# PKU-VCL-Geometry/GeoSplatting

Measured on AMD Instinct MI355X. Metric: fwd+bwd views/sec at 2M Gaussians, 800x800, higher is better.
Workload: dtype f32

## Files before the change

geosplatting_amd/csrc/gs_segsort_dev.h:

```cpp
#pragma once
#include <stdint.h>

#ifndef GS_SEGSORT_FN
#define GS_SEGSORT_FN __device__ __forceinline__
#endif

typedef unsigned long long gs_u64;

template <bool PAD>
GS_SEGSORT_FN int gs_seg_phys(int i) { return PAD ? i + (i >> 5) : i; }

template <bool F64>
GS_SEGSORT_FN gs_u64 gs_seg_inf() { return F64 ? 0x7ff0000000000000ull : ~0ull; }

template <bool F64>
GS_SEGSORT_FN void gs_seg_cx(gs_u64& a, gs_u64& b)
{
#if defined(__HIP_DEVICE_COMPILE__)
    if (F64) {
        const double x = __builtin_bit_cast(double, a), y = __builtin_bit_cast(double, b);
        double lo, hi;
        asm("v_min_f64 %0, %1, %2" : "=v"(lo) : "v"(x), "v"(y));
        asm("v_max_f64 %0, %1, %2" : "=v"(hi) : "v"(x), "v"(y));
        a = __builtin_bit_cast(gs_u64, lo); b = __builtin_bit_cast(gs_u64, hi);
        return;
    }
#endif
    const gs_u64 lo = a < b ? a : b, hi = a < b ? b : a;
    a = lo; b = hi;
}

template <int F, bool PAD, bool F64, bool GUARD>
GS_SEGSORT_FN void gs_seg_first(gs_u64* buf, int n, int P, int tid, int nthreads)
{
    constexpr int R = 1 << F;
    for (int v = tid; v < (P >> F); v += nthreads) {
        const int base = v << F;
        if (base >= n) break;
        gs_u64 e[R];
#pragma unroll
        for (int r = 0; r < R; ++r) e[r] = (!GUARD || base + r < n) ? buf[gs_seg_phys<PAD>(base + r)] : gs_seg_inf<F64>();
#pragma unroll
        for (int lgk = 1; lgk <= F; ++lgk) {
#pragma unroll
            for (int r = 0; r < R; ++r)
                if (r < (r ^ ((1 << lgk) - 1))) gs_seg_cx<F64>(e[r], e[r ^ ((1 << lgk) - 1)]);
#pragma unroll
            for (int s = lgk - 2; s >= 0; --s) {
#pragma unroll
                for (int r = 0; r < R; ++r)
                    if ((r & (1 << s)) == 0) gs_seg_cx<F64>(e[r], e[r | (1 << s)]);
            }
        }
#pragma unroll
        for (int r = 0; r < R; ++r) if (!GUARD || base + r < n) buf[gs_seg_phys<PAD>(base + r)] = e[r];
    }
}

template <int G, bool PAD, bool F64, bool GUARD>
GS_SEGSORT_FN void gs_seg_group(gs_u64* buf, int n, int P, int a, bool flip, int tid, int nthreads)
{
    constexpr int R = 1 << G, H = R >> 1;
    const int jmask = (1 << a) - 1;
    for (int v = tid; v < (P >> G); v += nthreads) {
        const int base = ((v >> a) << (a + G)) | (v & jmask);
        if (base >= n) break;
        const int base2 = flip ? (base ^ jmask) : base;
        gs_u64 e[R];
#pragma unroll
        for (int r = 0; r < R; ++r) {
            const int i = (r >= H ? base2 : base) + (r << a);
            e[r] = (!GUARD || i < n) ? buf[gs_seg_phys<PAD>(i)] : gs_seg_inf<F64>();
        }
        if (flip) {
#pragma unroll
            for (int r = 0; r < H; ++r) gs_seg_cx<F64>(e[r], e[R - 1 - r]);
        } else {
#pragma unroll
            for (int r = 0; r < H; ++r) gs_seg_cx<F64>(e[r], e[r + H]);
        }
#pragma unroll
        for (int s = G - 2; s >= 0; --s) {
#pragma unroll
            for (int r = 0; r < R; ++r)
                if ((r & (1 << s)) == 0) gs_seg_cx<F64>(e[r], e[r | (1 << s)]);
        }
#pragma unroll
        for (int r = 0; r < R; ++r) {
            const int i = (r >= H ? base2 : base) + (r << a);
            if (!GUARD || i < n) buf[gs_seg_phys<PAD>(i)] = e[r];
        }
    }
}

template <int GMAX, bool PAD, bool F64, bool GUARD>
GS_SEGSORT_FN void gs_seg_group_n(int g, gs_u64* buf, int n, int P, int a, bool flip, int tid, int nthreads)
{
    if (g == GMAX) gs_seg_group<GMAX, PAD, F64, GUARD>(buf, n, P, a, flip, tid, nthreads);
    else if constexpr (GMAX > 1) gs_seg_group_n<GMAX - 1, PAD, F64, GUARD>(g, buf, n, P, a, flip, tid, nthreads);
}

#define GS_SEG_SORT_BODY(GMAX, PAD, F64, GUARD, buf, n, P, tid, nthreads, BARRIER)                           \
    do {                                                                                                     \
        gs_seg_first<GMAX, PAD, F64, GUARD>(buf, n, P, tid, nthreads);                                       \
        BARRIER;                                                                                             \
        for (int k_ = 2 << (GMAX), lgk_ = (GMAX) + 1; k_ <= (P); k_ <<= 1, ++lgk_) {                         \
            int rem_ = lgk_;                                                                                 \
            bool flip_ = true;                                                                               \
            while (rem_ > 0) {                                                                               \
                const int g_ = flip_ ? ((rem_ - 1) % (GMAX)) + 1 : (GMAX);                                   \
                gs_seg_group_n<GMAX, PAD, F64, GUARD>(g_, buf, n, P, rem_ - g_, flip_, tid, nthreads);       \
                BARRIER;                                                                                     \
                rem_ -= g_;                                                                                  \
                flip_ = false;                                                                               \
            }                                                                                                \
        }                                                                                                    \
    } while (0)
```

geosplatting_amd/csrc/gs_sort.hip:

```cpp
#include "gs_common.h"
#include "gs_segsort_dev.h"

#include <cstdlib>
#include <cstring>

#define RS_THREADS 256
#define RS_WAVES 4
#define RS_ITEMS 8
#define RS_TILE (RS_THREADS * RS_ITEMS)
#define RS_WCHUNK (64 * RS_ITEMS)

typedef unsigned long long u64;

static int tile_bits(int tile_w, int tile_h)
{
    unsigned n = (unsigned)(tile_w * tile_h);
    int b = 0;
    while (n > 1) { n >>= 1; ++b; }
    return b + 1;
}

struct PairItem { u64 key; int32_t val; };
struct PairIn {
    const u64* keys; const int32_t* vals;
    __device__ __forceinline__ PairItem load(int64_t i) const { return PairItem{ keys[i], vals[i] }; }
};
struct PairOut {
    u64* keys; int32_t* vals;
    __device__ __forceinline__ void store(int64_t i, const PairItem& it) const { keys[i] = it.key; vals[i] = it.val; }
};
struct PairDigit {
    int shift; unsigned mask;
    __device__ __forceinline__ unsigned operator()(const PairItem& it) const { return (unsigned)(it.key >> shift) & mask; }
};

struct U2In {
    const uint2* p;
    __device__ __forceinline__ uint2 load(int64_t i) const { return p[i]; }
};
struct U2Out {
    uint2* p;
    __device__ __forceinline__ void store(int64_t i, const uint2& it) const { p[i] = it; }
};
struct DepthIn {
    const float* depths;
    __device__ __forceinline__ uint2 load(int64_t i) const { return make_uint2(__float_as_uint(depths[i]), (unsigned)i); }
};
struct XDigit {
    int shift; unsigned mask;
    __device__ __forceinline__ unsigned operator()(const uint2& it) const { return (it.x >> shift) & mask; }
};
struct FinalTiles {
    int32_t* tile_ids; int32_t* flatten_ids;
    __device__ __forceinline__ void store(int64_t i, const uint2& it) const
    {
        flatten_ids[i] = (int32_t)it.y;
        tile_ids[i] = (int32_t)it.x;
    }
};
struct FinalOut {
    u64* isect_ids; int32_t* flatten_ids; const float* depths;
    __device__ __forceinline__ void store(int64_t i, const uint2& it) const
    {
        flatten_ids[i] = (int32_t)it.y;
        isect_ids[i] = ((u64)it.x << 32) | (u64)__float_as_uint(depths[it.y]);
    }
};

template <typename Item, typename In, typename Digit>
__global__ void __launch_bounds__(RS_THREADS)
radix_hist_kernel(GsCount nc, In in, Digit digit, int nbins, int nblocks, unsigned* __restrict__ table)
{
    const int64_t n = gs_count(nc);
    __shared__ unsigned hist[256];
    hist[threadIdx.x] = 0u;
    __syncthreads();
    const int64_t base = (int64_t)blockIdx.x * RS_TILE;
#pragma unroll 4
    for (int k = 0; k < RS_ITEMS; ++k) {
        const int64_t i = base + (int64_t)k * RS_THREADS + threadIdx.x;
        if (i < n) atomicAdd(&hist[digit(in.load(i))], 1u);
    }
    __syncthreads();
    if ((int)threadIdx.x < nbins) table[(size_t)threadIdx.x * nblocks + blockIdx.x] = hist[threadIdx.x];
}

__global__ void __launch_bounds__(256)
radix_rowscan_kernel(int nblocks, unsigned* __restrict__ table, unsigned* __restrict__ row_total)
{
    __shared__ unsigned wsum[4];
    unsigned* row = table + (size_t)blockIdx.x * nblocks;
    const int lane = threadIdx.x & 63, wave = threadIdx.x >> 6;
    unsigned carry = 0u;
    for (int i0 = 0; i0 < nblocks; i0 += 256) {
        const int i = i0 + threadIdx.x;
        const unsigned v = i < nblocks ? row[i] : 0u;
        unsigned incl = v;
        incl = gs_wave_incl_scan(incl);
        if (lane == 63) wsum[wave] = incl;
        __syncthreads();
        unsigned before = 0u, all = 0u;
        for (int w = 0; w < 4; ++w) { if (w < wave) before += wsum[w]; all += wsum[w]; }
        if (i < nblocks) row[i] = carry + before + incl - v;
        carry += all;
        __syncthreads();
    }
    if (threadIdx.x == 0) row_total[blockIdx.x] = carry;
}

template <typename Item, typename In, typename Digit, typename Out, int NBITS>
__global__ void __launch_bounds__(RS_THREADS)
radix_scatter_kernel(GsCount nc, In in, Digit digit, int nblocks, const unsigned* __restrict__ table,
                     const unsigned* __restrict__ row_total, Out out)
{
    const int64_t n = gs_count(nc);
    constexpr int NB = 1 << NBITS;
    __shared__ unsigned cnt[RS_WAVES][NB];
    __shared__ unsigned dstart[NB];
    __shared__ unsigned gbase[NB];
    __shared__ Item stage[RS_TILE];
    const int lane = threadIdx.x & 63, wave = threadIdx.x >> 6;
    for (int i = threadIdx.x; i < RS_WAVES * NB; i += RS_THREADS) (&cnt[0][0])[i] = 0u;
    __syncthreads();
    const int64_t bbase = (int64_t)blockIdx.x * RS_TILE;
    const int64_t wbase = bbase + (int64_t)wave * RS_WCHUNK;
    const int n_here = (n - bbase) < RS_TILE ? (int)((n - bbase) > 0 ? (n - bbase) : 0) : RS_TILE;
    const u64 lane_lt = (1ull << lane) - 1ull;
    Item item[RS_ITEMS];
    unsigned dig[RS_ITEMS];
    unsigned rank[RS_ITEMS];
#pragma unroll
    for (int k = 0; k < RS_ITEMS; ++k) {
        const int64_t i = wbase + (int64_t)k * 64 + lane;
        const bool valid = i < n;
        if (valid) item[k] = in.load(i);
        const unsigned d = valid ? digit(item[k]) : 0u;
        u64 m = __ballot(valid);
#pragma unroll
        for (int b = 0; b < NBITS; ++b) {
            const bool bit = (d >> b) & 1u;
            const u64 bal = __ballot(bit);
            m &= bit ? bal : ~bal;
        }
        const unsigned old = cnt[wave][d];
        __builtin_amdgcn_wave_barrier();
        const unsigned r = __popcll(m & lane_lt);
        if (valid && r == 0u) cnt[wave][d] = old + (unsigned)__popcll(m);
        __builtin_amdgcn_fence(__ATOMIC_RELEASE, "wavefront");
        __builtin_amdgcn_wave_barrier();
        __builtin_amdgcn_fence(__ATOMIC_ACQUIRE, "wavefront");
        dig[k] = d;
        rank[k] = old + r;
    }
    __syncthreads();
    {
        const int d = threadIdx.x;
        unsigned tot = 0u;
        if (d < NB) for (int w = 0; w < RS_WAVES; ++w) tot += cnt[w][d];
        unsigned incl = tot;
        incl = gs_wave_incl_scan(incl);
        __shared__ unsigned wtot[RS_WAVES];
        if (lane == 63) wtot[wave] = incl;
        __syncthreads();
        unsigned before = 0u;
        for (int w = 0; w < wave; ++w) before += wtot[w];
        if (d < NB) dstart[d] = before + incl - tot;
        __syncthreads();
        const unsigned rt = d < NB ? row_total[d] : 0u;
        unsigned rincl = rt;
        rincl = gs_wave_incl_scan(rincl);
        if (lane == 63) wtot[wave] = rincl;
        __syncthreads();
        unsigned rbefore = 0u;
        for (int w = 0; w < wave; ++w) rbefore += wtot[w];
        if (d < NB) gbase[d] = rbefore + rincl - rt + table[(size_t)d * nblocks + blockIdx.x];
    }
    __syncthreads();
#pragma unroll
    for (int k = 0; k < RS_ITEMS; ++k) {
        const int64_t i = wbase + (int64_t)k * 64 + lane;
        if (i < n) {
            const unsigned d = dig[k];
            unsigned off = dstart[d] + rank[k];
            for (int w = 0; w < wave; ++w) off += cnt[w][d];
            stage[off] = item[k];
        }
    }
    __syncthreads();
#pragma unroll 4
    for (int k = 0; k < RS_ITEMS; ++k) {
        const int p = k * RS_THREADS + (int)threadIdx.x;
        if (p < n_here) {
            const Item it = stage[p];
            const unsigned d = digit(it);
            out.store((int64_t)gbase[d] + (int64_t)(p - (int)dstart[d]), it);
        }
    }
}

template <typename Item, typename In, typename Digit, typename Out>
static int radix_pass(GsCount nc, In in, Digit digit, Out out, int nbits, unsigned* table, hipStream_t s)
{
    const int64_t n = nc.n;
    const int nblocks = (int)((n + RS_TILE - 1) / RS_TILE);
    const int nbins = 1 << nbits;
    unsigned* row_total = table + (size_t)256 * nblocks;
    hipLaunchKernelGGL((radix_hist_kernel<Item, In, Digit>), dim3(nblocks), dim3(RS_THREADS), 0, s, nc, in, digit, nbins, nblocks, table);
    GS_CHECK_LAUNCH();
    hipLaunchKernelGGL(radix_rowscan_kernel, dim3(nbins), dim3(256), 0, s, nblocks, table, row_total);
    GS_CHECK_LAUNCH();
    switch (nbits) {
#define RS_CASE(B) case B: hipLaunchKernelGGL((radix_scatter_kernel<Item, In, Digit, Out, B>), dim3(nblocks), dim3(RS_THREADS), 0, s, nc, in, digit, nblocks, table, row_total, out); break;
        RS_CASE(1) RS_CASE(2) RS_CASE(3) RS_CASE(4) RS_CASE(5) RS_CASE(6) RS_CASE(7) RS_CASE(8)
#undef RS_CASE
        default: gs_set_error("radix_pass: bad digit width %d", nbits); return GS_EINVAL;
    }
    GS_CHECK_LAUNCH();
    return GS_OK;
}

static size_t align256(size_t x) { return (x + 255) & ~(size_t)255; }
static size_t table_bytes(int64_t n) { return align256(((size_t)256 * (size_t)((n + RS_TILE - 1) / RS_TILE + 1) + 512) * sizeof(unsigned)); }

extern "C" size_t gs_sort_ws_bytes(int64_t n_isects, int tile_w, int tile_h)
{
    if (n_isects <= 0) return 0;
    (void)tile_w; (void)tile_h;
    return table_bytes(n_isects) + align256((size_t)n_isects * 8) + align256((size_t)n_isects * 4) + 256;
}

extern "C" int gs_isect_sort(int64_t n_isects, const int64_t* isect_ids, const int32_t* flatten_ids,
                             int64_t* isect_ids_sorted, int32_t* flatten_ids_sorted, int tile_w, int tile_h,
                             void* ws, size_t ws_bytes, void* stream)
{
    GS_CHECK_ARG(n_isects >= 0 && tile_w > 0 && tile_h > 0, "bad sizes");
    if (n_isects == 0) return GS_OK;
    GS_CHECK_ARG(ws != nullptr, "workspace must not be NULL");
    if (ws_bytes < gs_sort_ws_bytes(n_isects, tile_w, tile_h)) { gs_set_error("gs_isect_sort: workspace too small"); return GS_ENOSPC; }
    hipStream_t s = (hipStream_t)stream;
    char* p = (char*)ws;
    unsigned* table = (unsigned*)p; p += table_bytes(n_isects);
    u64* tk = (u64*)p; p += align256((size_t)n_isects * 8);
    int32_t* tv = (int32_t*)p;
    const int end_bit = 32 + tile_bits(tile_w, tile_h);
    const int npass = (end_bit + 7) / 8;
    const u64* src_k = (const u64*)isect_ids; const int32_t* src_v = flatten_ids;
    for (int pass = 0; pass < npass; ++pass) {
        const int shift = pass * 8;
        const int nbits = (end_bit - shift) < 8 ? (end_bit - shift) : 8;
        const bool to_out = ((npass - 1 - pass) % 2) == 0;
        u64* dk = to_out ? (u64*)isect_ids_sorted : tk;
        int32_t* dv = to_out ? flatten_ids_sorted : tv;
        const int rc = radix_pass<PairItem>(GsCount{ n_isects, nullptr }, PairIn{ src_k, src_v }, PairDigit{ shift, (1u << nbits) - 1u }, PairOut{ dk, dv }, nbits, table, s);
        if (rc != GS_OK) return rc;
        src_k = dk; src_v = dv;
    }
    return GS_OK;
}

__device__ __forceinline__ void tile_range_sorted(float mx, float my, int radius, int tile_size, int tw, int th,
                                                  int& x0, int& y0, int& x1, int& y1)
{
#pragma clang fp contract(off)
    const float ts = (float)tile_size;
    const float tr = (float)radius / ts;
    const float tx = mx / ts, ty = my / ts;
    const float fx0 = floorf(tx - tr), fy0 = floorf(ty - tr);
    const float fx1 = ceilf(tx + tr), fy1 = ceilf(ty + tr);
    x0 = fx0 < 0.0f ? 0 : (fx0 > (float)tw ? tw : (int)fx0);
    y0 = fy0 < 0.0f ? 0 : (fy0 > (float)th ? th : (int)fy0);
    x1 = fx1 < 0.0f ? 0 : (fx1 > (float)tw ? tw : (int)fx1);
    y1 = fy1 < 0.0f ? 0 : (fy1 > (float)th ? th : (int)fy1);
}

#define EM_THREADS 256
#define EM_PER 4
#define EM_LOOK 4
#define EM_TILE (EM_THREADS * EM_PER)

__global__ void __launch_bounds__(256)
tile_rect_kernel(GsCount vc, const float* __restrict__ means2d, const int32_t* __restrict__ radii, int tile_size, int tile_w, int tile_h,
                 uint2* __restrict__ rect)
{
    const int V = (int)gs_count(vc);
    const int v = blockIdx.x * blockDim.x + threadIdx.x;
    if (v >= V) return;
    const float2 m = *reinterpret_cast<const float2*>(means2d + 2 * (size_t)v);
    int x0 = 0, y0 = 0, x1 = 0, y1 = 0;
    const int r = radii[v];
    if (r > 0) tile_range_sorted(m.x, m.y, r, tile_size, tile_w, tile_h, x0, y0, x1, y1);
    rect[v] = make_uint2((unsigned)x0 | ((unsigned)y0 << 16), (unsigned)x1 | ((unsigned)y1 << 16));
}
__device__ __forceinline__ unsigned rect_count(uint2 q)
{
    const int w = (int)(q.y & 0xffffu) - (int)(q.x & 0xffffu), h = (int)(q.y >> 16) - (int)(q.x >> 16);
    return (w > 0 && h > 0) ? (unsigned)(w * h) : 0u;
}

static size_t bf_state_bytes(int V) { return align256(16 + 2 * (size_t)((V + EM_TILE - 1) / EM_TILE + 1) * sizeof(u64)); }

extern "C" size_t gs_isect_bin_ws_bytes(int V, int64_t n_isects, int tile_w, int tile_h)
{
    (void)tile_w; (void)tile_h;
    const size_t v = V > 0 ? (size_t)V : 1, n = n_isects > 0 ? (size_t)n_isects : 1;
    const size_t tb = table_bytes((int64_t)(v > n ? v : n));
    return tb + 3 * align256(v * 8) + bf_state_bytes((int)v) + 2 * align256(n * 8) + 256;
}

__global__ void capacity_check_kernel(const long long* __restrict__ counts, long long v_cap, long long i_cap, long long* __restrict__ status)
{
    if (threadIdx.x != 0 || blockIdx.x != 0) return;
    const long long V = counts[0], I = counts[1];
    if (V > v_cap || I > i_cap) {
        status[0] = GS_ENOSPC;
        if (I > status[1]) status[1] = I;
        if (V > status[2]) status[2] = V;
    }
}

static int isect_bin_impl(int V, const float* means2d, const int32_t* radii, const float* depths, int64_t n_isects,
                          const long long* counts_dev, int tile_size, int tile_w, int tile_h, int64_t* isect_ids_sorted,
                          int32_t* flatten_ids_sorted, void* ws, size_t ws_bytes, void* stream, int32_t* tile_ids_sorted);

extern "C" int gs_isect_bin(int V, const float* means2d, const int32_t* radii, const float* depths,
                            const int32_t* tiles_per_gauss, int64_t n_isects, int tile_size, int tile_w, int tile_h,
                            int64_t* isect_ids_sorted, int32_t* flatten_ids_sorted, void* ws, size_t ws_bytes, void* stream)
{
    (void)tiles_per_gauss;
    return isect_bin_impl(V, means2d, radii, depths, n_isects, nullptr, tile_size, tile_w, tile_h, isect_ids_sorted, flatten_ids_sorted,
                          ws, ws_bytes, stream, nullptr);
}

extern "C" int gs_isect_bin_cap(int V_cap, const float* means2d, const int32_t* radii, const float* depths, const int64_t* counts_dev,
                                int64_t n_isects_cap, int tile_size, int tile_w, int tile_h, int64_t* isect_ids_sorted,
                                int32_t* flatten_ids_sorted, void* ws, size_t ws_bytes, int64_t* status_dev, void* stream)
{
    GS_CHECK_ARG(counts_dev != nullptr && status_dev != nullptr, "counts_dev / status_dev must not be NULL");
    hipLaunchKernelGGL(capacity_check_kernel, dim3(1), dim3(64), 0, (hipStream_t)stream, (const long long*)counts_dev, (long long)V_cap,
                       (long long)n_isects_cap, (long long*)status_dev);
    GS_CHECK_LAUNCH();
    return isect_bin_impl(V_cap, means2d, radii, depths, n_isects_cap, (const long long*)counts_dev, tile_size, tile_w, tile_h,
                          isect_ids_sorted, flatten_ids_sorted, ws, ws_bytes, stream, nullptr);
}

extern "C" int gs_isect_bin_tiles_cap(int V_cap, const float* means2d, const int32_t* radii, const float* depths, const int64_t* counts_dev,
                                      int64_t n_isects_cap, int tile_size, int tile_w, int tile_h, int32_t* tile_ids_sorted,
                                      int32_t* flatten_ids_sorted, void* ws, size_t ws_bytes, int64_t* status_dev, void* stream)
{
    GS_CHECK_ARG(counts_dev != nullptr && status_dev != nullptr && tile_ids_sorted != nullptr, "counts_dev / status_dev / tile_ids_sorted must not be NULL");
    hipLaunchKernelGGL(capacity_check_kernel, dim3(1), dim3(64), 0, (hipStream_t)stream, (const long long*)counts_dev, (long long)V_cap,
                       (long long)n_isects_cap, (long long*)status_dev);
    GS_CHECK_LAUNCH();
    return isect_bin_impl(V_cap, means2d, radii, depths, n_isects_cap, (const long long*)counts_dev, tile_size, tile_w, tile_h,
                          nullptr, flatten_ids_sorted, ws, ws_bytes, stream, tile_ids_sorted);
}

struct KeyIn {
    const unsigned* keys;
    __device__ __forceinline__ uint2 load(int64_t i) const { return make_uint2(keys[i], (unsigned)i); }
};
#define BF_HIST_MAX 8192

__global__ void __launch_bounds__(256)
bin_setup_kernel(unsigned* __restrict__ state, int n_state_words,
                 const long long* __restrict__ counts, long long v_cap, long long i_cap, long long* __restrict__ status)
{
    const int i = blockIdx.x * blockDim.x + threadIdx.x, stride = gridDim.x * blockDim.x;
    for (int k = i; k < n_state_words; k += stride) state[k] = 0u;
    if (i == 0 && counts != nullptr && status != nullptr) {
        const long long V = counts[0], I = counts[1];
        if (V > v_cap || I > i_cap) {
            status[0] = GS_ENOSPC;
            if (I > status[1]) status[1] = I;
            if (V > status[2]) status[2] = V;
        }
    }
}

#define BF_VALID (1ull << 63)
#define BF_SPIN_LIMIT (1 << 22)

__global__ void __launch_bounds__(EM_THREADS)
emit_chained_kernel(GsCount vc, const uint2* __restrict__ order, const uint2* __restrict__ rect, unsigned* __restrict__ ctrl,
                    u64* __restrict__ desc, int n_blocks, int tile_w, uint2* __restrict__ items, unsigned item_cap,
                    long long* __restrict__ status )
{
    const int V = (int)gs_count(vc);
    __shared__ unsigned ws[EM_THREADS / 64];
    __shared__ unsigned s_block;
    __shared__ unsigned long long s_base;
    const int lane = threadIdx.x & 63, wave = threadIdx.x >> 6;
    if (threadIdx.x == 0) s_block = atomicAdd(ctrl, 1u);
    __syncthreads();
    const int block = (int)s_block;
    u64* agg = desc; u64* pre = desc + n_blocks;
    const int r0 = block * EM_TILE + (int)threadIdx.x * EM_PER;
    int v[EM_PER]; unsigned c[EM_PER]; uint2 q[EM_PER];
    unsigned mine = 0u;
#pragma unroll
    for (int k = 0; k < EM_PER; ++k) {
        const int r = r0 + k;
        v[k] = r < V ? (int)order[r].y : -1;
        q[k] = v[k] >= 0 ? rect[v[k]] : make_uint2(0u, 0u);
        c[k] = rect_count(q[k]);
        mine += c[k];
    }
    unsigned incl = mine;
    incl = gs_wave_incl_scan(incl);
    if (lane == 63) ws[wave] = incl;
    __syncthreads();
    unsigned before = 0u, total = 0u;
    for (int w = 0; w < EM_THREADS / 64; ++w) { if (w < wave) before += ws[w]; total += ws[w]; }
    if (wave == 0) {
        unsigned long long acc = 0ull;
        if (block > 0) {
            if (lane == 0) __hip_atomic_store(&agg[block], (u64)total | BF_VALID, __ATOMIC_RELAXED, __HIP_MEMORY_SCOPE_AGENT);
            int pos = block - 1;
            bool done = false;
            while (!done) {
                u64 pv[EM_LOOK], av[EM_LOOK];
#pragma unroll
                for (int j = 0; j < EM_LOOK; ++j) {
                    const int idx = pos - 64 * j - lane;
                    pv[j] = av[j] = 0ull;
                    if (idx >= 0) {
                        pv[j] = __hip_atomic_load(&pre[idx], __ATOMIC_RELAXED, __HIP_MEMORY_SCOPE_AGENT);
                        av[j] = __hip_atomic_load(&agg[idx], __ATOMIC_RELAXED, __HIP_MEMORY_SCOPE_AGENT);
                    }
                }
#pragma unroll
                for (int j = 0; j < EM_LOOK; ++j) {
                    if (done) break;
                    const int idx = pos - 64 * j - lane;
                    bool isP = idx < 0;
                    u64 val = 0ull;
                    if (idx >= 0) {
                        int spins = 0;
                        for (;;) {
                            if (pv[j] & BF_VALID) { isP = true; val = pv[j]; break; }
                            if (av[j] & BF_VALID) { val = av[j]; break; }
                            if (++spins > BF_SPIN_LIMIT) { atomicExch(ctrl + 1, 1u); if (status) status[0] = GS_ENOSPC; break; }
                            __builtin_amdgcn_s_sleep(2);
                            pv[j] = __hip_atomic_load(&pre[idx], __ATOMIC_RELAXED, __HIP_MEMORY_SCOPE_AGENT);
                            av[j] = __hip_atomic_load(&agg[idx], __ATOMIC_RELAXED, __HIP_MEMORY_SCOPE_AGENT);
                        }
                    }
                    const u64 pmask = __ballot(isP);
                    const int first = pmask ? __builtin_ctzll(pmask) : 64;
                    if (lane <= first) acc += val & ~BF_VALID;
                    if (pmask) done = true;
                }
                pos -= 64 * EM_LOOK;
            }
        }
        const unsigned long long base = gs_wave_sum_u64(acc);
        if (lane == 0) {
            __hip_atomic_store(&pre[block], (u64)(base + total) | BF_VALID, __ATOMIC_RELAXED, __HIP_MEMORY_SCOPE_AGENT);
            s_base = base;
        }
    }
    __syncthreads();
    unsigned long long cur = s_base + before + incl - mine;
#pragma unroll
    for (int k = 0; k < EM_PER; ++k) {
        if (v[k] < 0 || c[k] == 0u) continue;
        const int x0 = (int)(q[k].x & 0xffffu), y0 = (int)(q[k].x >> 16), x1 = (int)(q[k].y & 0xffffu), y1 = (int)(q[k].y >> 16);
        for (int i = y0; i < y1; ++i)
            for (int j = x0; j < x1; ++j) {
                const unsigned t = (unsigned)(i * tile_w + j);
                if (cur < (unsigned long long)item_cap) items[cur] = make_uint2(t, (unsigned)v[k]);
                ++cur;
            }
    }
}

#define SEG_CLASSES 3
#define SEG_CAP0 2048
#define SEG_CAP1 4096
#define SEG_CAP2 16384
#define SEG_GMAX 4
#define SEG_THREADS(cap) ((cap) >> SEG_GMAX > 1024 ? 1024 : ((cap) >> SEG_GMAX))
#define SEG_BINS 64
static size_t seg_lds_bytes(int cap) { return (size_t)(cap + (cap >> 5) + 1) * sizeof(u64); }

extern "C" int gs_isect_bin_front_classes(int* caps, int max)
{
    const int c[SEG_CLASSES] = { SEG_CAP0, SEG_CAP1, SEG_CAP2 };
    for (int i = 0; i < SEG_CLASSES && i < max; ++i) if (caps) caps[i] = c[i];
    return SEG_CLASSES;
}

struct SegLists { unsigned* count; int32_t* lists; };

__device__ __forceinline__ int seg_class(unsigned len) { return len <= SEG_CAP0 ? 0 : (len <= SEG_CAP1 ? 1 : (len <= SEG_CAP2 ? 2 : 3)); }
__device__ __forceinline__ int seg_bin(unsigned len)
{
    const int l2 = 31 - __clz((int)len);
    const int half = l2 > 0 ? (int)((len >> (l2 - 1)) & 1u) : 0;
    return SEG_BINS - 1 - (2 * l2 + half);
}

__global__ void __launch_bounds__(1024)
tile_offsets_scan_kernel(int n_tiles, const unsigned* __restrict__ tile_counts, GsCount nc, int32_t* __restrict__ offsets, SegLists sl)
{
    __shared__ unsigned wsum[16];
    __shared__ unsigned s_bin[(SEG_CLASSES + 1) * SEG_BINS];
    const unsigned n = (unsigned)gs_count(nc);
    const int lane = threadIdx.x & 63, wave = threadIdx.x >> 6;
    if (sl.count && threadIdx.x < (SEG_CLASSES + 1) * SEG_BINS) s_bin[threadIdx.x] = 0u;
    __syncthreads();
    unsigned carry = 0u;
    for (int i0 = 0; i0 < n_tiles; i0 += 1024) {
        const int i = i0 + threadIdx.x;
        const unsigned v = i < n_tiles ? tile_counts[i] : 0u;
        unsigned incl = v;
        incl = gs_wave_incl_scan(incl);
        if (lane == 63) wsum[wave] = incl;
        __syncthreads();
        unsigned before = 0u, all = 0u;
        for (int w = 0; w < 16; ++w) { if (w < wave) before += wsum[w]; all += wsum[w]; }
        if (i < n_tiles) {
            const unsigned o = carry + before + incl - v;
            const unsigned beg = o < n ? o : n, end = o + v < n ? o + v : n;
            offsets[i] = (int32_t)beg;
            if (sl.count && end > beg) atomicAdd(&s_bin[seg_class(end - beg) * SEG_BINS + seg_bin(end - beg)], 1u);
        }
        carry += all;
        __syncthreads();
    }
    if (!sl.count) return;
    if (wave <= SEG_CLASSES) {
        const unsigned v = s_bin[wave * SEG_BINS + lane];
        const unsigned incl = gs_wave_incl_scan(v);
        s_bin[wave * SEG_BINS + lane] = incl - v;
        if (lane == 63) sl.count[wave] = incl;
    }
    __syncthreads();
    for (int i = threadIdx.x; i < n_tiles; i += 1024) {
        const unsigned beg = (unsigned)offsets[i];
        unsigned end = n;
        if (i + 1 < n_tiles) end = (unsigned)__hip_atomic_load(&offsets[i + 1], __ATOMIC_RELAXED, __HIP_MEMORY_SCOPE_WORKGROUP);
        if (end > beg) {
            const int c = seg_class(end - beg);
            const unsigned pos = atomicAdd(&s_bin[c * SEG_BINS + seg_bin(end - beg)], 1u);
            sl.lists[(size_t)c * n_tiles + pos] = i;
        }
    }
}

#define SC_THREADS 512
#define SC_PER 8
#define SC_TILE (SC_THREADS * SC_PER)

__global__ void __launch_bounds__(SC_THREADS)
bin_scatter_kernel(GsCount vc, const unsigned* __restrict__ keys, const uint2* __restrict__ rects, unsigned key_mask, u64 item_bias, int tile_w, int tile_h,
                   const int32_t* __restrict__ offsets, unsigned* __restrict__ cursor, u64* __restrict__ items, unsigned item_cap)
{
    extern __shared__ unsigned s_pos[];
    const int V = (int)gs_count(vc);
    const int n_tiles = tile_w * tile_h;
    const int s0 = (int)blockIdx.x * SC_TILE + (int)threadIdx.x;
    if ((long long)blockIdx.x * SC_TILE >= V) return;
    for (int t = threadIdx.x; t < n_tiles; t += SC_THREADS) s_pos[t] = 0u;
    unsigned key[SC_PER]; uint2 q[SC_PER];
#pragma unroll
    for (int k = 0; k < SC_PER; ++k) {
        const int v = s0 + k * SC_THREADS;
        const int vv = v < V ? v : V - 1;
        key[k] = keys[vv];
        q[k] = rects[vv];
        if (v >= V) q[k] = make_uint2(0u, 0u);
    }
#pragma unroll
    for (int k = 0; k < SC_PER; ++k) {
        int x1 = (int)(q[k].y & 0xffffu), y1 = (int)(q[k].y >> 16);
        x1 = x1 < tile_w ? x1 : tile_w; y1 = y1 < tile_h ? y1 : tile_h;
        q[k].y = (unsigned)x1 | ((unsigned)y1 << 16);
    }
    __syncthreads();
#pragma unroll
    for (int k = 0; k < SC_PER; ++k) {
        const int x0 = (int)(q[k].x & 0xffffu), y0 = (int)(q[k].x >> 16), x1 = (int)(q[k].y & 0xffffu), y1 = (int)(q[k].y >> 16);
        for (int i = y0; i < y1; ++i)
            for (int j = x0; j < x1; ++j) atomicAdd(&s_pos[i * tile_w + j], 1u);
    }
    __syncthreads();
    for (int t0 = threadIdx.x; t0 < n_tiles; t0 += 4 * SC_THREADS) {
        unsigned c[4], o[4], b[4];
#pragma unroll
        for (int u = 0; u < 4; ++u) {
            const int t = t0 + u * SC_THREADS;
            c[u] = t < n_tiles ? s_pos[t] : 0u;
            o[u] = c[u] ? (unsigned)offsets[t] : 0u;
        }
#pragma unroll
        for (int u = 0; u < 4; ++u) b[u] = c[u] ? atomicAdd(&cursor[t0 + u * SC_THREADS], c[u]) : 0u;
#pragma unroll
        for (int u = 0; u < 4; ++u) if (c[u]) s_pos[t0 + u * SC_THREADS] = o[u] + b[u];
    }
    __syncthreads();
#pragma unroll
    for (int k = 0; k < SC_PER; ++k) {
        const int x0 = (int)(q[k].x & 0xffffu), y0 = (int)(q[k].x >> 16), x1 = (int)(q[k].y & 0xffffu), y1 = (int)(q[k].y >> 16);
        const u64 item = item_bias | ((u64)(key[k] & key_mask) << 31) | (u64)(unsigned)(s0 + k * SC_THREADS);
        for (int i = y0; i < y1; ++i)
            for (int j = x0; j < x1; ++j) {
                const unsigned pos = atomicAdd(&s_pos[i * tile_w + j], 1u);
                if (pos < item_cap) items[pos] = item;
            }
    }
}

template <int THREADS, bool GLOBAL, bool F64>
__global__ void __launch_bounds__(THREADS)
seg_sort_kernel(const int32_t* __restrict__ list, const unsigned* __restrict__ list_count, int n_tiles, const int32_t* __restrict__ offsets,
                GsCount ic, GsCount vc, u64* items, int32_t* __restrict__ flat)
{
    extern __shared__ u64 s_seg[];
    if (blockIdx.x >= *list_count) return;
    const int t = list[blockIdx.x];
    const int n_all = (int)gs_count(ic);
    const int beg = offsets[t], end = t + 1 < n_tiles ? offsets[t + 1] : n_all;
    const int n = end - beg;
    if (n <= 0) return;
    const long long V = gs_count(vc);
    const unsigned vmax = V > 0 ? (unsigned)(V - 1) : 0u;
    const int tid = threadIdx.x;
    int P = 1 << SEG_GMAX;
    while (P < n) P <<= 1;
    u64* buf = GLOBAL ? items + beg : s_seg;
    if (!GLOBAL) {
        for (int i = tid; i < P; i += THREADS) s_seg[gs_seg_phys<true>(i)] = i < n ? items[beg + i] : gs_seg_inf<F64>();
        __syncthreads();
    }
    GS_SEG_SORT_BODY(SEG_GMAX, !GLOBAL, F64, GLOBAL, buf, n, P, tid, THREADS, __syncthreads());
    for (int i = tid; i < n; i += THREADS) {
        const unsigned slot = (unsigned)buf[gs_seg_phys<!GLOBAL>(i)] & 0x7fffffffu;
        flat[beg + i] = (int32_t)(slot < vmax ? slot : vmax);
    }
}

__global__ void __launch_bounds__(256)
bin_offsets_tiles_kernel(GsCount nc, const int32_t* __restrict__ tiles, int n_tiles, int32_t* __restrict__ offsets)
{
    const int64_t n = gs_count(nc);
    const int64_t i = (int64_t)blockIdx.x * blockDim.x + threadIdx.x;
    if (n == 0 && i == 0)
        for (int t = 0; t < n_tiles; ++t) offsets[t] = 0;
    if (i >= n) return;
    const int cur = tiles[i];
    if (i == 0) {
        for (int t = 0; t <= cur && t < n_tiles; ++t) offsets[t] = 0;
    } else {
        const int prev = tiles[i - 1];
        for (int t = prev + 1; t <= cur && t < n_tiles; ++t) offsets[t] = (int32_t)i;
    }
    if (i == n - 1)
        for (int t = cur + 1; t < n_tiles; ++t) offsets[t] = (int32_t)n;
}


static size_t tf_state_words(int n_tiles) { return (size_t)n_tiles + SEG_CLASSES + 1; }
static size_t tf_ws_bytes(int64_t n_isects, int n_tiles)
{
    return align256(tf_state_words(n_tiles) * 4) + align256((size_t)(SEG_CLASSES + 1) * n_tiles * 4) + align256((size_t)n_isects * 8) + 256;
}
static size_t bf_radix_ws_bytes(size_t v, size_t n)
{
    return table_bytes((int64_t)(v > n ? v : n)) + 2 * align256(v * 8) + 2 * align256(n * 8) + bf_state_bytes((int)v) + align256(n * 4) + 256;
}

extern "C" size_t gs_isect_bin_front_ws_bytes(int V, int64_t n_isects, int tile_w, int tile_h)
{
    const size_t v = V > 0 ? (size_t)V : 1, n = n_isects > 0 ? (size_t)n_isects : 1;
    const int64_t n_tiles = (int64_t)tile_w * tile_h;
    if (n_tiles > 0 && n_tiles <= BF_HIST_MAX) return tf_ws_bytes((int64_t)n, (int)n_tiles);
    return bf_radix_ws_bytes(v, n);
}

static int bin_front_tile_first(int V, const uint32_t* depth_keys, const uint32_t* tile_rects, const uint32_t* tile_counts,
                                const int64_t* counts_dev, int64_t n_isects, int key_bits, int tile_w, int tile_h, int32_t* flatten_ids_sorted,
                                int32_t* isect_offsets, void* ws, int64_t* status_dev, hipStream_t s)
{
    const int n_tiles = tile_w * tile_h;
    const GsCount vc{ (long long)V, (const long long*)counts_dev }, ic{ (long long)n_isects, counts_dev ? (const long long*)counts_dev + 1 : nullptr };
    char* p = (char*)ws;
    unsigned* cursor = (unsigned*)p;
    unsigned* class_count = cursor + n_tiles; p += align256(tf_state_words(n_tiles) * 4);
    int32_t* lists = (int32_t*)p; p += align256((size_t)(SEG_CLASSES + 1) * n_tiles * 4);
    u64* items = (u64*)p;
    const int n_state_words = (int)tf_state_words(n_tiles);
    hipLaunchKernelGGL(bin_setup_kernel, dim3(gs_cdiv(n_state_words, 256) < 64 ? gs_cdiv(n_state_words, 256) : 64), dim3(256), 0, s, cursor,
                       n_state_words, (const long long*)counts_dev, (long long)V, (long long)n_isects, (long long*)status_dev);
    GS_CHECK_LAUNCH();
    hipLaunchKernelGGL(tile_offsets_scan_kernel, dim3(1), dim3(1024), 0, s, n_tiles, (const unsigned*)tile_counts, ic, isect_offsets,
                       SegLists{ class_count, lists });
    GS_CHECK_LAUNCH();
    const bool f64 = key_bits == 24;
    hipLaunchKernelGGL(bin_scatter_kernel, dim3(gs_cdiv(V, SC_TILE)), dim3(SC_THREADS), (size_t)n_tiles * 4, s, vc,
                       (const unsigned*)depth_keys, (const uint2*)tile_rects, f64 ? 0xffffffu : 0xffffffffu, f64 ? (1ull << 62) : 0ull, tile_w, tile_h,
                       (const int32_t*)isect_offsets, cursor, items, (unsigned)n_isects);
    GS_CHECK_LAUNCH();
    GS_CHECK_HIP(hipFuncSetAttribute((const void*)seg_sort_kernel<SEG_THREADS(SEG_CAP2), false, false>, hipFuncAttributeMaxDynamicSharedMemorySize, (int)seg_lds_bytes(SEG_CAP2)));
    GS_CHECK_HIP(hipFuncSetAttribute((const void*)seg_sort_kernel<SEG_THREADS(SEG_CAP2), false, true>, hipFuncAttributeMaxDynamicSharedMemorySize, (int)seg_lds_bytes(SEG_CAP2)));
    const int caps[SEG_CLASSES + 1] = { 0, SEG_CAP0, SEG_CAP1, SEG_CAP2 };
    for (int c = 0; c <= SEG_CLASSES; ++c) {
        const int64_t most = n_isects / (caps[c] + 1);
        const int grid = (int)(most < n_tiles ? most : n_tiles);
        if (grid == 0) continue;
        const int32_t* list = lists + (size_t)c * n_tiles;
#define SEG_LAUNCH1(T, G, F, LDS) hipLaunchKernelGGL((seg_sort_kernel<T, G, F>), dim3(grid), dim3(T), LDS, s, list, (const unsigned*)(class_count + c), n_tiles, \
                                                     (const int32_t*)isect_offsets, ic, vc, items, flatten_ids_sorted)
#define SEG_LAUNCH(T, G, LDS) do { if (f64) SEG_LAUNCH1(T, G, true, LDS); else SEG_LAUNCH1(T, G, false, LDS); } while (0)
        if (c == 0) SEG_LAUNCH(SEG_THREADS(SEG_CAP0), false, seg_lds_bytes(SEG_CAP0));
        else if (c == 1) SEG_LAUNCH(SEG_THREADS(SEG_CAP1), false, seg_lds_bytes(SEG_CAP1));
        else if (c == 2) SEG_LAUNCH(SEG_THREADS(SEG_CAP2), false, seg_lds_bytes(SEG_CAP2));
        else SEG_LAUNCH(1024, true, 0);
#undef SEG_LAUNCH
#undef SEG_LAUNCH1
        GS_CHECK_LAUNCH();
    }
    return GS_OK;
}

extern "C" int gs_isect_bin_front(int V_cap, const uint32_t* depth_keys, const uint32_t* tile_rects, const uint32_t* tile_counts,
                                  const int64_t* counts_dev, int64_t n_isects_cap, int key_bits, int tile_w, int tile_h, int32_t* flatten_ids_sorted,
                                  int32_t* isect_offsets, void* ws, size_t ws_bytes, int64_t* status_dev, void* stream)
{
    const int V = V_cap;
    const int64_t n_isects = n_isects_cap;
    GS_CHECK_ARG(V >= 0 && n_isects >= 0 && tile_w > 0 && tile_h > 0 && (key_bits == 24 || key_bits == 32), "bad sizes or key width");
    GS_CHECK_ARG(n_isects < (1ll << 31), "n_isects must fit int32");
    GS_CHECK_ARG((int64_t)tile_w * tile_h < (1ll << 24) && tile_w < 65536 && tile_h < 65536, "tile grid too large");
    GS_CHECK_ARG(isect_offsets != nullptr && (counts_dev == nullptr || status_dev != nullptr), "null argument");
    hipStream_t s = (hipStream_t)stream;
    const int n_tiles = tile_w * tile_h;
    if (V == 0 || n_isects == 0) { GS_CHECK_HIP(gs_zero_async(isect_offsets, sizeof(int32_t) * (size_t)n_tiles, s)); return GS_OK; }
    GS_CHECK_ARG(depth_keys != nullptr && tile_rects != nullptr && flatten_ids_sorted != nullptr && ws != nullptr, "null argument");
    if (tile_counts != nullptr && n_tiles <= BF_HIST_MAX) {
        if (ws_bytes < tf_ws_bytes(n_isects, n_tiles)) { gs_set_error("gs_isect_bin_front: workspace too small"); return GS_ENOSPC; }
        return bin_front_tile_first(V, depth_keys, tile_rects, tile_counts, counts_dev, n_isects, key_bits, tile_w, tile_h, flatten_ids_sorted,
                                    isect_offsets, ws, status_dev, s);
    }
    if (ws_bytes < bf_radix_ws_bytes((size_t)V, (size_t)n_isects)) { gs_set_error("gs_isect_bin_front: workspace too small for the radix path (no tile_counts)"); return GS_ENOSPC; }
    const GsCount vc{ (long long)V, (const long long*)counts_dev }, ic{ (long long)n_isects, counts_dev ? (const long long*)counts_dev + 1 : nullptr };
    char* p = (char*)ws;
    unsigned* table = (unsigned*)p; p += table_bytes((int64_t)V > n_isects ? (int64_t)V : n_isects);
    uint2* da = (uint2*)p; p += align256((size_t)V * 8);
    uint2* db = (uint2*)p; p += align256((size_t)V * 8);
    uint2* ia = (uint2*)p; p += align256((size_t)n_isects * 8);
    uint2* ib = (uint2*)p; p += align256((size_t)n_isects * 8);
    unsigned* state = (unsigned*)p; p += bf_state_bytes(V);
    int32_t* tile_ids = (int32_t*)p;
    const int eblocks = (V + EM_TILE - 1) / EM_TILE;
    const int n_state_words = (int)(bf_state_bytes(V) / 4);
    hipLaunchKernelGGL(bin_setup_kernel, dim3(gs_cdiv(n_state_words, 256) < 64 ? gs_cdiv(n_state_words, 256) : 64),
                       dim3(256), 0, s, state, n_state_words, (const long long*)counts_dev,
                       (long long)V_cap, (long long)n_isects_cap, (long long*)status_dev);
    GS_CHECK_LAUNCH();
    int rc = radix_pass<uint2>(vc, KeyIn{ depth_keys }, XDigit{ 0, 255u }, U2Out{ da }, 8, table, s);
    if (rc != GS_OK) return rc;
    rc = radix_pass<uint2>(vc, U2In{ da }, XDigit{ 8, 255u }, U2Out{ db }, 8, table, s);
    if (rc != GS_OK) return rc;
    rc = radix_pass<uint2>(vc, U2In{ db }, XDigit{ 16, 255u }, U2Out{ da }, 8, table, s);
    if (rc != GS_OK) return rc;
    const uint2* order = da;
    if (key_bits == 32) {
        rc = radix_pass<uint2>(vc, U2In{ da }, XDigit{ 24, 255u }, U2Out{ db }, 8, table, s);
        if (rc != GS_OK) return rc;
        order = db;
    }
    unsigned* ctrl = state; u64* desc = (u64*)((char*)state + 16);
    hipLaunchKernelGGL(emit_chained_kernel, dim3(eblocks), dim3(EM_THREADS), 0, s, vc, order, (const uint2*)tile_rects, ctrl, desc,
                       eblocks + 1, tile_w, ia, (unsigned)n_isects, (long long*)status_dev);
    GS_CHECK_LAUNCH();
    int tb = 0;
    while ((1 << tb) < n_tiles) ++tb;
    if (tb < 1) tb = 1;
    const int npass = (tb + 7) / 8, width = (tb + npass - 1) / npass;
    uint2* src = ia; uint2* dst = ib;
    for (int pass = 0; pass < npass; ++pass) {
        const int shift = pass * width;
        const int nbits = (tb - shift) < width ? (tb - shift) : width;
        if (pass == npass - 1)
            rc = radix_pass<uint2>(ic, U2In{ src }, XDigit{ shift, (1u << nbits) - 1u }, FinalTiles{ tile_ids, flatten_ids_sorted }, nbits, table, s);
        else
            rc = radix_pass<uint2>(ic, U2In{ src }, XDigit{ shift, (1u << nbits) - 1u }, U2Out{ dst }, nbits, table, s);
        if (rc != GS_OK) return rc;
        uint2* t = src; src = dst; dst = t;
    }
    hipLaunchKernelGGL(bin_offsets_tiles_kernel, dim3(gs_cdiv(n_isects, 256)), dim3(256), 0, s, ic, tile_ids, n_tiles, isect_offsets);
    GS_CHECK_LAUNCH();
    return GS_OK;
}

static int isect_bin_impl(int V, const float* means2d, const int32_t* radii, const float* depths, int64_t n_isects,
                          const long long* counts_dev, int tile_size, int tile_w, int tile_h, int64_t* isect_ids_sorted,
                          int32_t* flatten_ids_sorted, void* ws, size_t ws_bytes, void* stream, int32_t* tile_ids_sorted)
{
    const GsCount vc{ (long long)V, counts_dev }, ic{ (long long)n_isects, counts_dev ? counts_dev + 1 : nullptr };
    GS_CHECK_ARG(V >= 0 && n_isects >= 0 && tile_size > 0 && tile_w > 0 && tile_h > 0, "bad sizes");
    GS_CHECK_ARG(n_isects < (1ll << 31), "n_isects must fit int32");
    GS_CHECK_ARG((int64_t)tile_w * tile_h < (1ll << 24), "more than 2^24 tiles");
    if (V == 0 || n_isects == 0) return GS_OK;
    GS_CHECK_ARG(ws != nullptr, "workspace must not be NULL");
    if (ws_bytes < gs_isect_bin_ws_bytes(V, n_isects, tile_w, tile_h)) { gs_set_error("gs_isect_bin: workspace too small"); return GS_ENOSPC; }
    hipStream_t s = (hipStream_t)stream;
    char* p = (char*)ws;
    unsigned* table = (unsigned*)p; p += table_bytes((int64_t)V > n_isects ? (int64_t)V : n_isects);
    uint2* da = (uint2*)p; p += align256((size_t)V * 8);
    uint2* db = (uint2*)p; p += align256((size_t)V * 8);
    uint2* rect = (uint2*)p; p += align256((size_t)V * 8);
    const int eblocks = (V + EM_TILE - 1) / EM_TILE;
    unsigned* state = (unsigned*)p; p += bf_state_bytes(V);
    uint2* ia = (uint2*)p; p += align256((size_t)n_isects * 8);
    uint2* ib = (uint2*)p; p += align256((size_t)n_isects * 8);
    int tb = 0;
    while ((1 << tb) < tile_w * tile_h) ++tb;
    if (tb < 1) tb = 1;
    const int npass = (tb + 7) / 8, width = (tb + npass - 1) / npass;
    int rc = GS_OK;
    rc = radix_pass<uint2>(vc, DepthIn{ depths }, XDigit{ 0, 255u }, U2Out{ da }, 8, table, s);
    if (rc != GS_OK) return rc;
    rc = radix_pass<uint2>(vc, U2In{ da }, XDigit{ 8, 255u }, U2Out{ db }, 8, table, s);
    if (rc != GS_OK) return rc;
    rc = radix_pass<uint2>(vc, U2In{ db }, XDigit{ 16, 255u }, U2Out{ da }, 8, table, s);
    if (rc != GS_OK) return rc;
    rc = radix_pass<uint2>(vc, U2In{ da }, XDigit{ 24, 255u }, U2Out{ db }, 8, table, s);
    if (rc != GS_OK) return rc;
    GS_CHECK_ARG(tile_w < 65536 && tile_h < 65536, "tile grid too large");
    hipLaunchKernelGGL(tile_rect_kernel, dim3(gs_cdiv(V, 256)), dim3(256), 0, s, vc, means2d, radii, tile_size, tile_w, tile_h, rect);
    GS_CHECK_LAUNCH();
    {
        const int n_state_words = (int)(bf_state_bytes(V) / 4);
        hipLaunchKernelGGL(bin_setup_kernel, dim3(gs_cdiv(n_state_words, 256) < 64 ? gs_cdiv(n_state_words, 256) : 64), dim3(256), 0, s, state,
                           n_state_words, (const long long*)nullptr, 0ll, 0ll, (long long*)nullptr);
        GS_CHECK_LAUNCH();
        hipLaunchKernelGGL(emit_chained_kernel, dim3(eblocks), dim3(EM_THREADS), 0, s, vc, (const uint2*)db, (const uint2*)rect, state,
                           (u64*)((char*)state + 16), eblocks + 1, tile_w, ia, (unsigned)n_isects, (long long*)nullptr);
        GS_CHECK_LAUNCH();
    }
    uint2* src = ia; uint2* dst = ib;
    for (int pass = 0; pass < npass; ++pass) {
        const int shift = pass * width;
        const int nbits = (tb - shift) < width ? (tb - shift) : width;
        if (pass == npass - 1 && tile_ids_sorted != nullptr)
            rc = radix_pass<uint2>(ic, U2In{ src }, XDigit{ shift, (1u << nbits) - 1u },
                                   FinalTiles{ tile_ids_sorted, flatten_ids_sorted }, nbits, table, s);
        else if (pass == npass - 1)
            rc = radix_pass<uint2>(ic, U2In{ src }, XDigit{ shift, (1u << nbits) - 1u },
                                   FinalOut{ (u64*)isect_ids_sorted, flatten_ids_sorted, depths }, nbits, table, s);
        else
            rc = radix_pass<uint2>(ic, U2In{ src }, XDigit{ shift, (1u << nbits) - 1u }, U2Out{ dst }, nbits, table, s);
        if (rc != GS_OK) return rc;
        uint2* t = src; src = dst; dst = t;
    }
    return GS_OK;
}
```

Measured before the change: 754.9.

## Replace large-segment size classes with chunked hybrid LDS/global bitonic sort

Segments longer than 2048 now go through a single class sorted by a new hybrid kernel. It sorts 8K-element chunks in LDS, then merges across chunks with global-memory steps and finishes each merge stage inside LDS, so tiles above 16K no longer need a pure-global bitonic sort. The bin_setup kernel is removed: its cursor zeroing and capacity/status check move into tile_offsets_scan_kernel, saving one launch. The tradeoff is that mid-size segments (2K–16K), which were previously sorted entirely in LDS, may now pay extra global passes.

```diff
diff --git a/geosplatting_amd/csrc/gs_segsort_dev.h b/geosplatting_amd/csrc/gs_segsort_dev.h
--- a/geosplatting_amd/csrc/gs_segsort_dev.h
+++ b/geosplatting_amd/csrc/gs_segsort_dev.h
@@ -116,3 +116,58 @@
             }                                                                                                \
         }                                                                                                    \
     } while (0)
+
+template <int GMAX, int LGC, int NT, bool F64, class Barrier, class Emit>
+GS_SEGSORT_FN void gs_seg_hybrid(gs_u64* lds, gs_u64* g, int n, int tid, Barrier bar, Emit emit)
+{
+    static_assert(LGC > GMAX, "a chunk holds more than one group");
+    constexpr int C = 1 << LGC;
+    if (n <= C) {
+        int P = 1 << GMAX;
+        while (P < n) P <<= 1;
+        for (int i = tid; i < P; i += NT) lds[gs_seg_phys<true>(i)] = i < n ? g[i] : gs_seg_inf<F64>();
+        bar();
+        GS_SEG_SORT_BODY(GMAX, true, F64, false, lds, n, P, tid, NT, bar());
+        for (int i = tid; i < n; i += NT) emit(i, lds[gs_seg_phys<true>(i)]);
+        return;
+    }
+    int lgP = LGC + 1;
+    while ((1ll << lgP) < (long long)n) ++lgP;
+    for (int cb = 0; cb < n; cb += C) {
+        const int nl = n - cb < C ? n - cb : C;
+        int Pl = 1 << GMAX;
+        while (Pl < nl) Pl <<= 1;
+        for (int i = tid; i < Pl; i += NT) lds[gs_seg_phys<true>(i)] = i < nl ? g[cb + i] : gs_seg_inf<F64>();
+        bar();
+        GS_SEG_SORT_BODY(GMAX, true, F64, false, lds, nl, Pl, tid, NT, bar());
+        for (int i = tid; i < nl; i += NT) g[cb + i] = lds[gs_seg_phys<true>(i)];
+        bar();
+    }
+    const int P = 1 << lgP;
+    for (int lgk = LGC + 1; lgk <= lgP; ++lgk) {
+        int rem = lgk;
+        bool flip = true;
+        while (rem > LGC) {
+            const int gg = flip ? ((rem - LGC - 1) % GMAX) + 1 : GMAX;
+            gs_seg_group_n<GMAX, false, F64, true>(gg, g, n, P, rem - gg, flip, tid, NT);
+            bar();
+            rem -= gg;
+            flip = false;
+        }
+        const bool last = lgk == lgP;
+        for (int cb = 0; cb < n; cb += C) {
+            const int nl = n - cb < C ? n - cb : C;
+            for (int i = tid; i < C; i += NT) lds[gs_seg_phys<true>(i)] = i < nl ? g[cb + i] : gs_seg_inf<F64>();
+            bar();
+            for (int r = LGC; r > 0;) {
+                const int gg = ((r - 1) % GMAX) + 1;
+                gs_seg_group_n<GMAX, true, F64, false>(gg, lds, nl, C, r - gg, false, tid, NT);
+                bar();
+                r -= gg;
+            }
+            if (last) { for (int i = tid; i < nl; i += NT) emit(cb + i, lds[gs_seg_phys<true>(i)]); }
+            else      { for (int i = tid; i < nl; i += NT) g[cb + i] = lds[gs_seg_phys<true>(i)]; }
+            bar();
+        }
+    }
+}
diff --git a/geosplatting_amd/csrc/gs_sort.hip b/geosplatting_amd/csrc/gs_sort.hip
--- a/geosplatting_amd/csrc/gs_sort.hip
+++ b/geosplatting_amd/csrc/gs_sort.hip
@@ -474,25 +474,29 @@
     }
 }
 
-#define SEG_CLASSES 3
+#define SEG_CLASSES 2
 #define SEG_CAP0 2048
-#define SEG_CAP1 4096
-#define SEG_CAP2 16384
+#define SEG_LG_CHUNK 13
+#define SEG_CHUNK (1 << SEG_LG_CHUNK)
 #define SEG_GMAX 4
-#define SEG_THREADS(cap) ((cap) >> SEG_GMAX > 1024 ? 1024 : ((cap) >> SEG_GMAX))
+#define SEG_THREADS(cap) ((cap) >> SEG_GMAX)
 #define SEG_BINS 64
 static size_t seg_lds_bytes(int cap) { return (size_t)(cap + (cap >> 5) + 1) * sizeof(u64); }
 
 extern "C" int gs_isect_bin_front_classes(int* caps, int max)
 {
-    const int c[SEG_CLASSES] = { SEG_CAP0, SEG_CAP1, SEG_CAP2 };
-    for (int i = 0; i < SEG_CLASSES && i < max; ++i) if (caps) caps[i] = c[i];
-    return SEG_CLASSES;
-}
-
-struct SegLists { unsigned* count; int32_t* lists; };
-
-__device__ __forceinline__ int seg_class(unsigned len) { return len <= SEG_CAP0 ? 0 : (len <= SEG_CAP1 ? 1 : (len <= SEG_CAP2 ? 2 : 3)); }
+    const int c[2] = { SEG_CAP0, SEG_CHUNK };
+    for (int i = 0; i < 2 && i < max; ++i) if (caps) caps[i] = c[i];
+    return 2;
+}
+
+struct SegLists {
+    unsigned* count; int32_t* lists;
+    unsigned* cursor;
+    const long long* counts; long long v_cap, i_cap; long long* status;
+};
+
+__device__ __forceinline__ int seg_class(unsigned len) { return len <= SEG_CAP0 ? 0 : 1; }
 __device__ __forceinline__ int seg_bin(unsigned len)
 {
     const int l2 = 31 - __clz((int)len);
@@ -504,10 +508,18 @@
 tile_offsets_scan_kernel(int n_tiles, const unsigned* __restrict__ tile_counts, GsCount nc, int32_t* __restrict__ offsets, SegLists sl)
 {
     __shared__ unsigned wsum[16];
-    __shared__ unsigned s_bin[(SEG_CLASSES + 1) * SEG_BINS];
+    __shared__ unsigned s_bin[SEG_CLASSES * SEG_BINS];
     const unsigned n = (unsigned)gs_count(nc);
     const int lane = threadIdx.x & 63, wave = threadIdx.x >> 6;
-    if (sl.count && threadIdx.x < (SEG_CLASSES + 1) * SEG_BINS) s_bin[threadIdx.x] = 0u;
+    if (sl.count && threadIdx.x < SEG_CLASSES * SEG_BINS) s_bin[threadIdx.x] = 0u;
+    if (sl.count && threadIdx.x == 0 && sl.counts != nullptr && sl.status != nullptr) {
+        const long long V = sl.counts[0], I = sl.counts[1];
+        if (V > sl.v_cap || I > sl.i_cap) {
+            sl.status[0] = GS_ENOSPC;
+            if (I > sl.status[1]) sl.status[1] = I;
+            if (V > sl.status[2]) sl.status[2] = V;
+        }
+    }
     __syncthreads();
     unsigned carry = 0u;
     for (int i0 = 0; i0 < n_tiles; i0 += 1024) {
@@ -523,13 +535,14 @@
             const unsigned o = carry + before + incl - v;
             const unsigned beg = o < n ? o : n, end = o + v < n ? o + v : n;
             offsets[i] = (int32_t)beg;
+            if (sl.count) sl.cursor[i] = 0u;
             if (sl.count && end > beg) atomicAdd(&s_bin[seg_class(end - beg) * SEG_BINS + seg_bin(end - beg)], 1u);
         }
         carry += all;
         __syncthreads();
     }
     if (!sl.count) return;
-    if (wave <= SEG_CLASSES) {
+    if (wave < SEG_CLASSES) {
         const unsigned v = s_bin[wave * SEG_BINS + lane];
         const unsigned incl = gs_wave_incl_scan(v);
         s_bin[wave * SEG_BINS + lane] = incl - v;
@@ -611,7 +624,7 @@
     }
 }
 
-template <int THREADS, bool GLOBAL, bool F64>
+template <int THREADS, bool F64>
 __global__ void __launch_bounds__(THREADS)
 seg_sort_kernel(const int32_t* __restrict__ list, const unsigned* __restrict__ list_count, int n_tiles, const int32_t* __restrict__ offsets,
                 GsCount ic, GsCount vc, u64* items, int32_t* __restrict__ flat)
@@ -628,16 +641,34 @@
     const int tid = threadIdx.x;
     int P = 1 << SEG_GMAX;
     while (P < n) P <<= 1;
-    u64* buf = GLOBAL ? items + beg : s_seg;
-    if (!GLOBAL) {
-        for (int i = tid; i < P; i += THREADS) s_seg[gs_seg_phys<true>(i)] = i < n ? items[beg + i] : gs_seg_inf<F64>();
-        __syncthreads();
-    }
-    GS_SEG_SORT_BODY(SEG_GMAX, !GLOBAL, F64, GLOBAL, buf, n, P, tid, THREADS, __syncthreads());
+    for (int i = tid; i < P; i += THREADS) s_seg[gs_seg_phys<true>(i)] = i < n ? items[beg + i] : gs_seg_inf<F64>();
+    __syncthreads();
+    GS_SEG_SORT_BODY(SEG_GMAX, true, F64, false, s_seg, n, P, tid, THREADS, __syncthreads());
     for (int i = tid; i < n; i += THREADS) {
-        const unsigned slot = (unsigned)buf[gs_seg_phys<!GLOBAL>(i)] & 0x7fffffffu;
+        const unsigned slot = (unsigned)s_seg[gs_seg_phys<true>(i)] & 0x7fffffffu;
         flat[beg + i] = (int32_t)(slot < vmax ? slot : vmax);
     }
+}
+
+template <int THREADS, int LG_CHUNK, bool F64>
+__global__ void __launch_bounds__(THREADS)
+seg_sort_large_kernel(const int32_t* __restrict__ list, const unsigned* __restrict__ list_count, int n_tiles, const int32_t* __restrict__ offsets,
+                      GsCount ic, GsCount vc, u64* items, int32_t* __restrict__ flat)
+{
+    __shared__ u64 s_seg[(1 << LG_CHUNK) + (1 << (LG_CHUNK - 5)) + 1];
+    if (blockIdx.x >= *list_count) return;
+    const int t = list[blockIdx.x];
+    const int n_all = (int)gs_count(ic);
+    const int beg = offsets[t], end = t + 1 < n_tiles ? offsets[t + 1] : n_all;
+    const int n = end - beg;
+    if (n <= 0) return;
+    const long long V = gs_count(vc);
+    const unsigned vmax = V > 0 ? (unsigned)(V - 1) : 0u;
+    gs_seg_hybrid<SEG_GMAX, LG_CHUNK, THREADS, F64>(s_seg, items + beg, n, (int)threadIdx.x, [] { __syncthreads(); },
+        [=](int i, u64 w) {
+            const unsigned slot = (unsigned)w & 0x7fffffffu;
+            flat[beg + i] = (int32_t)(slot < vmax ? slot : vmax);
+        });
 }
 
 __global__ void __launch_bounds__(256)
@@ -660,10 +691,10 @@
 }
 
 
-static size_t tf_state_words(int n_tiles) { return (size_t)n_tiles + SEG_CLASSES + 1; }
+static size_t tf_state_words(int n_tiles) { return (size_t)n_tiles + SEG_CLASSES; }
 static size_t tf_ws_bytes(int64_t n_isects, int n_tiles)
 {
-    return align256(tf_state_words(n_tiles) * 4) + align256((size_t)(SEG_CLASSES + 1) * n_tiles * 4) + align256((size_t)n_isects * 8) + 256;
+    return align256(tf_state_words(n_tiles) * 4) + align256((size_t)SEG_CLASSES * n_tiles * 4) + align256((size_t)n_isects * 8) + 256;
 }
 static size_t bf_radix_ws_bytes(size_t v, size_t n)
 {
@@ -687,37 +718,32 @@
     char* p = (char*)ws;
     unsigned* cursor = (unsigned*)p;
     unsigned* class_count = cursor + n_tiles; p += align256(tf_state_words(n_tiles) * 4);
-    int32_t* lists = (int32_t*)p; p += align256((size_t)(SEG_CLASSES + 1) * n_tiles * 4);
+    int32_t* lists = (int32_t*)p; p += align256((size_t)SEG_CLASSES * n_tiles * 4);
     u64* items = (u64*)p;
-    const int n_state_words = (int)tf_state_words(n_tiles);
-    hipLaunchKernelGGL(bin_setup_kernel, dim3(gs_cdiv(n_state_words, 256) < 64 ? gs_cdiv(n_state_words, 256) : 64), dim3(256), 0, s, cursor,
-                       n_state_words, (const long long*)counts_dev, (long long)V, (long long)n_isects, (long long*)status_dev);
-    GS_CHECK_LAUNCH();
     hipLaunchKernelGGL(tile_offsets_scan_kernel, dim3(1), dim3(1024), 0, s, n_tiles, (const unsigned*)tile_counts, ic, isect_offsets,
-                       SegLists{ class_count, lists });
+                       SegLists{ class_count, lists, cursor, (const long long*)counts_dev, (long long)V, (long long)n_isects, (long long*)status_dev });
     GS_CHECK_LAUNCH();
     const bool f64 = key_bits == 24;
     hipLaunchKernelGGL(bin_scatter_kernel, dim3(gs_cdiv(V, SC_TILE)), dim3(SC_THREADS), (size_t)n_tiles * 4, s, vc,
                        (const unsigned*)depth_keys, (const uint2*)tile_rects, f64 ? 0xffffffu : 0xffffffffu, f64 ? (1ull << 62) : 0ull, tile_w, tile_h,
                        (const int32_t*)isect_offsets, cursor, items, (unsigned)n_isects);
     GS_CHECK_LAUNCH();
-    GS_CHECK_HIP(hipFuncSetAttribute((const void*)seg_sort_kernel<SEG_THREADS(SEG_CAP2), false, false>, hipFuncAttributeMaxDynamicSharedMemorySize, (int)seg_lds_bytes(SEG_CAP2)));
-    GS_CHECK_HIP(hipFuncSetAttribute((const void*)seg_sort_kernel<SEG_THREADS(SEG_CAP2), false, true>, hipFuncAttributeMaxDynamicSharedMemorySize, (int)seg_lds_bytes(SEG_CAP2)));
-    const int caps[SEG_CLASSES + 1] = { 0, SEG_CAP0, SEG_CAP1, SEG_CAP2 };
-    for (int c = 0; c <= SEG_CLASSES; ++c) {
+    const int caps[SEG_CLASSES] = { 0, SEG_CAP0 };
+    for (int c = 0; c < SEG_CLASSES; ++c) {
         const int64_t most = n_isects / (caps[c] + 1);
         const int grid = (int)(most < n_tiles ? most : n_tiles);
         if (grid == 0) continue;
         const int32_t* list = lists + (size_t)c * n_tiles;
-#define SEG_LAUNCH1(T, G, F, LDS) hipLaunchKernelGGL((seg_sort_kernel<T, G, F>), dim3(grid), dim3(T), LDS, s, list, (const unsigned*)(class_count + c), n_tiles, \
-                                                     (const int32_t*)isect_offsets, ic, vc, items, flatten_ids_sorted)
-#define SEG_LAUNCH(T, G, LDS) do { if (f64) SEG_LAUNCH1(T, G, true, LDS); else SEG_LAUNCH1(T, G, false, LDS); } while (0)
-        if (c == 0) SEG_LAUNCH(SEG_THREADS(SEG_CAP0), false, seg_lds_bytes(SEG_CAP0));
-        else if (c == 1) SEG_LAUNCH(SEG_THREADS(SEG_CAP1), false, seg_lds_bytes(SEG_CAP1));
-        else if (c == 2) SEG_LAUNCH(SEG_THREADS(SEG_CAP2), false, seg_lds_bytes(SEG_CAP2));
-        else SEG_LAUNCH(1024, true, 0);
+#define SEG_LAUNCH(KERNEL, T, LDS) hipLaunchKernelGGL(KERNEL, dim3(grid), dim3(T), LDS, s, list, (const unsigned*)(class_count + c), n_tiles, \
+                                                      (const int32_t*)isect_offsets, ic, vc, items, flatten_ids_sorted)
+        if (c == 0) {
+            if (f64) SEG_LAUNCH((seg_sort_kernel<SEG_THREADS(SEG_CAP0), true>), SEG_THREADS(SEG_CAP0), seg_lds_bytes(SEG_CAP0));
+            else SEG_LAUNCH((seg_sort_kernel<SEG_THREADS(SEG_CAP0), false>), SEG_THREADS(SEG_CAP0), seg_lds_bytes(SEG_CAP0));
+        } else {
+            if (f64) SEG_LAUNCH((seg_sort_large_kernel<SEG_THREADS(SEG_CHUNK), SEG_LG_CHUNK, true>), SEG_THREADS(SEG_CHUNK), 0);
+            else SEG_LAUNCH((seg_sort_large_kernel<SEG_THREADS(SEG_CHUNK), SEG_LG_CHUNK, false>), SEG_THREADS(SEG_CHUNK), 0);
+        }
 #undef SEG_LAUNCH
-#undef SEG_LAUNCH1
         GS_CHECK_LAUNCH();
     }
     return GS_OK;
```

Result: faster. 762.8, median of 6 (+1.1%).
